# etrigger/Parsip

Measured on AMD Instinct MI355X. Metric: Mcells/sec polygonized, 256^3 grid 32-prim BlobTree, at 1/2/4/8 MI355X, higher is better.
Workload: dtype f32

## Files before the change

include/parsip_gpu.h:

```cpp
#ifndef PARSIP_GPU_H
#define PARSIP_GPU_H

#ifdef __HIPCC_RTC__
typedef __SIZE_TYPE__ size_t;
#ifndef offsetof
#define offsetof(t, m) __builtin_offsetof(t, m)
#endif
#else
#include <stddef.h>
#include <stdint.h>
#endif

#ifdef __cplusplus
extern "C" {
#endif

#define PSGPU_GRID_DIM              8
#define PSGPU_CELLS_PER_MPU         7
#define PSGPU_ISO_VALUE             0.5f
#define PSGPU_ISO_DIST              0.45420206f
#define PSGPU_NORMAL_DELTA          0.001f
#define PSGPU_MIN_CELL_SIZE         0.01f
#define PSGPU_MAX_TREE_NODES        128
#define PSGPU_PRIM_MATRIX_STRIDE    12
// ... 150 lines not shown
int  psgpu_weld_times(psgpu_ctx* ctx, float* ms, int maxPhases, const char** names);

int  psgpu_download_stats(psgpu_ctx* ctx, PsMpuStats* stats);
int  psgpu_export_polympus(psgpu_ctx* ctx, PsMPU* mpus, uint32_t capacity, uint32_t* outCtMPUs);
int  psgpu_polygonize_mpus(psgpu_ctx* ctx, float cellsize, const PsSoaBlobPrims* prims,
                           const PsSoaPrimMatrices* matrices, const PsSoaBlobOps* ops,
                           PsMPU* mpus, uint32_t capacity, uint32_t* outCtMPUs,
                           PsMpuStats* statsOrNull);
int  psgpu_polygonize_mpus_ex(psgpu_ctx* ctx, float cellsize, const PsSoaBlobPrims* prims,
                              const PsSoaPrimMatrices* matrices, const PsSoaBlobOps* ops,
                              PsMPU* mpus, uint32_t capacity, uint32_t* outCtMPUs,
                              PsMpuStats* statsOrNull, PsMpuProcessStats* processStatsOrNull);
int  psgpu_download_process_stats(psgpu_ctx* ctx, PsMpuProcessStats* out);
int  psgpu_download_stamps(psgpu_ctx* ctx, uint64_t* out, uint32_t* cap);
int  psgpu_vertex_queue(psgpu_ctx* ctx, uint32_t* counts, uint32_t* recs, uint32_t capacity);
int  psgpu_print_thread_results(int ctAttempts, uint32_t* lpThreadProcessed, uint32_t* lpThreadCrossed,
                                uint32_t capacity, int print);
int  psgpu_thread_result_count(void);
int  psgpu_last_kernel_times(psgpu_ctx* ctx, float* ms, int maxKernels, const char** names);
int  psgpu_field_values(psgpu_ctx* ctx, const float* xyz, uint32_t n, int mode, float* out, float* colOut);
int  psgpu_download_spans(psgpu_ctx* ctx, uint64_t* out, uint32_t* runs);

int  psgpu_set_option(psgpu_ctx* ctx, int option, int64_t value);
#define PSGPU_OPT_KERNEL_TIMING 1
#define PSGPU_OPT_CULLING       2
#define PSGPU_OPT_DEBUG         9
#define PSGPU_OPT_VERTEX_BLOCKS_PER_CU 4
#define PSGPU_OPT_FINISH_BLOCKS_PER_CU 5
#define PSGPU_OPT_GRAPH         7
#define PSGPU_OPT_CAPACITY      6
#define PSGPU_OPT_BOUND        10
#define PSGPU_OPT_JIT           3
#define PSGPU_OPT_TIER_RUNS    18
#define PSGPU_OPT_STAMPS       12
#define PSGPU_OPT_SPANS        13
#define PSGPU_OPT_FINISH_QUAD  14
#define PSGPU_OPT_VERTEX_WIDE  15
#define PSGPU_OPT_TREE_SPLIT   16
#define PSGPU_OPT_SPLIT_MAX_QUEUED 17
#define PSGPU_OPT_FUSED_SURFACE 21
// ... 101 lines not shown
```

parsip_amd/csrc/psgpu_device.h:

```cpp
#pragma once
#include "psgpu_model.h"

namespace psgpu {

typedef const __attribute__((address_space(4))) DevModel* ModelPtr;
typedef const __attribute__((address_space(4))) DevPrim CPrim;
typedef const __attribute__((address_space(4))) DevOp COp;
typedef const __attribute__((address_space(4))) CubeTablesDev* TablePtr;
__device__ __forceinline__ ModelPtr as_const(const DevModel* m) { return (ModelPtr)m; }
__device__ __forceinline__ TablePtr as_const(const CubeTablesDev* t) { return (TablePtr)t; }

__device__ __forceinline__ Instr load_instr(ModelPtr M, int pc) {
    typedef const __attribute__((address_space(4))) uint32_t* CU32;
    const CU32 w = (CU32)(&M->instr[pc]);
    const uint32_t words[3] = {w[0], w[1], w[2]};
    Instr I;
    __builtin_memcpy(&I, words, 12);
    return I;
}

__device__ __forceinline__ float max_ref(float a, float b) { return a > b ? a : b; }
__device__ __forceinline__ float min_ref(float a, float b) { return a < b ? a : b; }
__device__ __forceinline__ float m01(bool c) { return c ? 1.0f : 0.0f; }
__device__ __forceinline__ int lane_id() { return __lane_id(); }
// ... 260 lines not shown
    case PSGPU_T_UNION: case PSGPU_T_INTERSECT:
        *wl = m01((v - lf) == 0.0f);
        *wr = m01((v - rf) == 0.0f);
        return true;
    case PSGPU_T_DIF: case PSGPU_T_SMOOTHDIF:
        *wl = m01(lf == v);
        *wr = m01((1.0f - rf) == v);
        return true;
    default:
        return false;
    }
}

struct CullMask {
    uint64_t lo, hi;
};

struct CullLanes {
    CullSeg s[2];
    bool two;
};

__device__ __forceinline__ CullSeg load_cullseg(ModelPtr M, int i) {
    typedef const __attribute__((address_space(4))) float* CF;
    const CF f = (CF)(&M->cull[i]);
    CullSeg S;
    S.a[0] = f[0]; S.a[1] = f[1]; S.a[2] = f[2];
    S.u[0] = f[3]; S.u[1] = f[4]; S.u[2] = f[5];
    S.invUU = f[6]; S.radius = f[7];
    S.tmin = f[8]; S.tmax = f[9]; S.axisClear = f[10]; S.pad = f[11];
    return S;
// ... 485 lines not shown
    const bool vOf = __shfl(valid ? 1 : 0, lane * 8 & 63) != 0;
    const bool pass = lane < 8 && ((queue8 >> lane) & 1u);
    if (lane < 8 && vOf) {
        p.passed[mOf - p.mpuBegin] = (uint8_t)(((flags8 >> lane) & 1u) + ((queue8 >> lane) & 1u));
        if (!pass) p.counts[mOf - p.mpuBegin] = 0ull;
        if (p.mpuTicks) mpu_ticks_s1(p, mOf - p.mpuBegin, tick0);
    }
    if (flags8 == 0u) return;
    const uint32_t shard = W / (p.pShardCap / 8u);
    if (lane == 1 && proven8 != 0u) atomicAdd(&p.ctr->shard[shard].b, (uint32_t)__popc(proven8));
    if (queue8 == 0u) return;
    const uint32_t qsel = FRONT ? (blockIdx.x & 7u) : shard;
    const uint32_t qbase = FRONT ? qsel * p.fqCap : shard * p.pShardCap;
    uint32_t baseAtomic = 0;
    if (lane == 0) baseAtomic = atomicAdd(&p.ctr->shard[qsel].p, (uint32_t)__popc(queue8));
    uint64_t mLo = 0ull, mHi = 0ull;
    if (p.cull) {
        const float eg = 7.0f * p.cs + 0.001f;
        for (uint32_t qm = queue8; qm != 0u; qm &= qm - 1u) {
            const int q = __builtin_ctz(qm);
            const float ox = __int_as_float(__builtin_amdgcn_readlane(__float_as_int(o[0]), 8 * q));
            const float oy = __int_as_float(__builtin_amdgcn_readlane(__float_as_int(o[1]), 8 * q));
            const float oz = __int_as_float(__builtin_amdgcn_readlane(__float_as_int(o[2]), 8 * q));
            const CullMask g = cull_mask_from(cl, ox, oy, oz, ox + eg, oy + eg, oz + eg);
            const uint32_t wq = lane_value(mOf, q) - p.mpuBegin;
            if (lane == 0) {
                p.mpuMasks[2 * wq] = g.lo;
                p.mpuMasks[2 * wq + 1] = g.hi;
            }
            if (lane == q) {
                mLo = g.lo;
                mHi = g.hi;
            }
        }
    }
    asm volatile("" : "+v"(baseAtomic) : "v"(mLo));
    const uint32_t base = lane_value(baseAtomic, 0);
    if (pass) {
        const uint32_t slotq = qbase + base + (uint32_t)__popc(queue8 & ((1u << lane) - 1u));
        if (FRONT) {
            __hip_atomic_store(&p.pq[slotq], mOf, __ATOMIC_RELAXED, __HIP_MEMORY_SCOPE_AGENT);
            if (p.cull) {
                __hip_atomic_store(&p.pqMask[2 * slotq], mLo, __ATOMIC_RELAXED, __HIP_MEMORY_SCOPE_AGENT);
                __hip_atomic_store(&p.pqMask[2 * slotq + 1], mHi, __ATOMIC_RELAXED, __HIP_MEMORY_SCOPE_AGENT);
            }
        } else {
            p.pq[slotq] = mOf;
            if (p.cull) {
                p.pqMask[2 * slotq] = mLo;
                p.pqMask[2 * slotq + 1] = mHi;
            }
        }
    }
    phase_stamp(p, 3, 8192u);
    if constexpr (FRONT) {
        asm volatile("s_waitcnt vmcnt(0)" ::: "memory");
        if (pass) {
            const uint32_t slotq = qbase + base + (uint32_t)__popc(queue8 & ((1u << lane) - 1u));
            __hip_atomic_store(&p.fqReady[slotq], front_tag(p), __ATOMIC_RELAXED, __HIP_MEMORY_SCOPE_AGENT);
        }
    }
}

#ifndef PSGPU_S2_N
#define PSGPU_S2_N 8
// ... 95 lines not shown
        if (blk * (uint32_t)MPB >= pcount) return;
        live = d < pcount;
        if (live) {
            const uint32_t pshard = (uint32_t)__popcll(ballot(incl <= d));
            const uint32_t pidx = d - (pshard ? sIncl[pshard - 1] : 0u);
            slotq = uniform(pshard * p.pShardCap + pidx);
        }
    }
    uint32_t m = 0, w = 0;
    float o[3] = {0.0f, 0.0f, 0.0f};
    CullMask cm{0ull, 0ull};
    if (live) {
        if (FRONT) {
            m = uniform(__hip_atomic_load(&p.pq[slotq], __ATOMIC_RELAXED, __HIP_MEMORY_SCOPE_AGENT));
            if (p.cull) {
                cm.lo = uniform64(__hip_atomic_load(&p.pqMask[2 * slotq], __ATOMIC_RELAXED, __HIP_MEMORY_SCOPE_AGENT));
                cm.hi = uniform64(__hip_atomic_load(&p.pqMask[2 * slotq + 1], __ATOMIC_RELAXED, __HIP_MEMORY_SCOPE_AGENT));
            }
        } else {
            m = uniform(p.pq[slotq]);
            if (p.cull) {
                cm.lo = uniform64(p.pqMask[2 * slotq]);
                cm.hi = uniform64(p.pqMask[2 * slotq + 1]);
            }
        }
        *item = m;
        w = m - p.mpuBegin;
        mpu_origin(p, m, o);
    }
    phase_stamp(p, 1);
    unsigned char* base = smem + slot * kLdsMpu;
    uint16_t* edgeVid = reinterpret_cast<uint16_t*>(base + kLdsEdge);
    uint8_t* cellCfg = base + kLdsCfg;
    uint16_t* cellV = reinterpret_cast<uint16_t*>(base + kLdsVbase);
    uint16_t* cellT = reinterpret_cast<uint16_t*>(base + kLdsTbase);
    uint64_t* sIns = reinterpret_cast<uint64_t*>(base + kLdsIns);
    uint32_t* sQ = reinterpret_cast<uint32_t*>(base + kLdsQ);
    EV ev(M, reinterpret_cast<float*>(smem + kLdsWaveSlots + wave * p.slotsPerLane * 64 * 4) + lane);
// ... 361 lines not shown
#pragma unroll
        for (int i = 0; i < 8; ++i) {
            runV += (uint32_t)ch.c[i];
            runT += (uint32_t)(ch.c[i] >> 32);
            out[i] = (uint64_t)runV | ((uint64_t)runT << 32);
        }
#pragma unroll
        for (int i = 0; i < 8; ++i)
            if (e0 + i < hi) p.offs[e0 + i + 1] = out[i];
        carryV += totV;
        carryT += totT;
    }
}

__device__ __forceinline__ CullMask cull_mask_mpus(const Params& p, uint32_t w) {
    CullMask cm{~0ull, ~0ull};
    bool todo = true;
    for (;;) {
        const uint64_t b = ballot(todo);
        if (b == 0ull) break;
        const uint32_t w0 = lane_value(w, (int)__builtin_ctzll(b));
        cm.lo &= p.mpuMasks[2 * w0];
        cm.hi &= p.mpuMasks[2 * w0 + 1];
        if (w == w0) todo = false;
    }
    return cm;
}

struct EdgeSeg {
    float e[3], d[3];
};
__device__ __forceinline__ EdgeSeg edge_segment(const Params& p, uint32_t w, uint32_t key) {
    float o[3];
    mpu_origin(p, w + p.mpuBegin, o);
    const int sx = key & 7, sy = (key >> 3) & 7, sz = (key >> 6) & 7, ax = (key >> 9) & 3;
    const float cs = p.cs;
    EdgeSeg E;
    E.e[0] = o[0] + cs * (float)sx;
// ... 624 lines not shown
```

parsip_amd/csrc/psgpu_host.cpp:

```cpp
#include <hip/hip_runtime.h>

#include <atomic>
#include <algorithm>
#include <numeric>
#include <cmath>
#include <cstdio>
#include <cstdlib>
#include <cstring>
#include <ctime>
#include <functional>
#include <limits>
#include <memory>
#include <chrono>
#include <mutex>
#include <string>
#include <thread>
#include <vector>

#include "../../include/parsip_gpu.h"
#include "psgpu_internal.h"
#include "psgpu_launch.h"


using namespace psgpu;
// ... 368 lines not shown
    return (size_t)bd[0] * bd[1] * bd[2];
}

uint32_t front_sub_cap(uint32_t blocks, uint32_t mpb) { return 8u * mpb * ((blocks + 7u) / 8u); }
uint32_t front_cap(size_t bricks) {
    const uint32_t b = (uint32_t)bricks;
    return std::max(front_sub_cap((b + 1u) / 2u, 2u), front_sub_cap((b + 3u) / 4u, 4u));
}

int ensure_buffers(psgpu_ctx* c, uint32_t mpuCount) {
    const size_t n = std::max<uint32_t>(mpuCount, 1);
    c->pShardCap = 8u * (uint32_t)((brick_count(c) + kShards - 1) / kShards);
    const size_t fq = 8 * front_cap(brick_count(c));
    const size_t nq = std::max<size_t>((size_t)c->pShardCap * kShards, fq);
    PSGPU_CHECK(grow(c->pq, c->capList, nq));
    PSGPU_CHECK(grow(c->pqMask, c->capPqMask, nq * 2));
    if (fq > c->capFq) {
        PSGPU_CHECK(grow(c->fqReady, c->capFq, fq));
        PSGPU_CHECK(hipMemset(c->fqReady, 0, c->capFq * sizeof(uint32_t)));
    }
    PSGPU_CHECK(grow(c->counts, c->capCounts, n));
    PSGPU_CHECK(grow(c->passed, c->capPassed, n));
    PSGPU_CHECK(grow(c->mpuMasks, c->capMasks, 2 * n));
    PSGPU_CHECK(grow(c->offs, c->capOff, n + 1));
    PSGPU_CHECK(grow(c->vk, c->capVk, (size_t)c->vShardCap * kShards));
    PSGPU_CHECK(grow(c->vp, c->capVp, (size_t)c->vShardCap * kShards));
    PSGPU_CHECK(grow(c->tq, c->capTq, (size_t)c->tShardCap * kShards));
    size_t capV2 = c->capV, capV3 = c->capV;
    PSGPU_CHECK(grow(c->pos, c->capV, (size_t)c->vcap * 3));
    PSGPU_CHECK(grow(c->nrm, capV2, (size_t)c->vcap * 3));
    PSGPU_CHECK(grow(c->col, capV3, (size_t)c->vcap * 3));
    PSGPU_CHECK(grow(c->tris, c->capT, (size_t)c->tcap * 3));
    if (c->mpuTicksOpt) PSGPU_CHECK(grow(c->mpuTicks, c->capTicks, 4 * n));
    return PSGPU_RET_SUCCESS;
}

bool use_split(const psgpu_ctx* c) {
    if (!c->jit || !c->jit->precheckS || !c->splittable) return false;
// ... 42 lines not shown
    if (use_front(c)) {
        const uint32_t sub = !c->haveQueued ? p.fqCap
                             : (c->lastSubMax ? c->lastSubMax : (c->lastQueued + 7u) / 8u) + c->lastQueued / 32u + 32u;
        const uint32_t rows = (std::min(sub, p.fqCap) + mpb - 1u) / mpb;
        p.mpuBlocks = 8u * std::max(1u, rows);
    }
    if (c->debug & (1 << 20)) p.mpuBlocks = use_front(c) ? 8u : 1u;
    p.scanChunks = (c->mpuCount + kScanItems * kScanMaxBlocks - 1) / (kScanItems * kScanMaxBlocks);
    if (p.scanChunks == 0) p.scanChunks = 1;
    p.scanBlocks = (c->mpuCount + kScanItems * p.scanChunks - 1) / (kScanItems * p.scanChunks);
    p.scanStatus = c->scanStatus + (size_t)c->parity * kScanMaxBlocks;
    p.scanStatusNext = c->scanStatus + (size_t)(c->parity ^ 1u) * kScanMaxBlocks;
    p.counts = c->counts;
    p.passed = c->passed;
    p.bound = (c->bound && c->jit && c->model.boundable) ? 1u : 0u;
    p.mpuMasks = c->mpuMasks;
    p.offs = c->offs;
    p.vk = c->vk;
    p.vp = c->vp;
    p.vShardCap = c->vShardCap;
    p.tq = c->tq;
    p.tShardCap = c->tShardCap;
    p.pos = c->pos;
    p.nrm = c->nrm;
    p.col = c->col;
    p.tris = c->tris;
    p.vCap = c->vcap;
    p.tCap = c->tcap;
    p.ctr = c->ctr + c->parity;
    p.ctrNext = c->ctr + (c->parity ^ 1u);
// ... 472 lines not shown
            return PSGPU_RET_DEVICE_ERROR;
        }
    }
    {
        DevCounters init[2];
        memset(init, 0, sizeof(init));
        init[0].firstOverflow = init[1].firstOverflow = 0x7fffffff;
        if (hipMemcpy(c->ctr, init, sizeof(init), hipMemcpyHostToDevice) != hipSuccess) {
            psgpu_destroy(c);
            return PSGPU_RET_DEVICE_ERROR;
        }
    }
    for (int i = 0; i <= kNumKernels; ++i) (void)hipEventCreate(&c->ev[i]);
    const char* cullEnv = getenv("PSGPU_CULL");
    if (cullEnv) c->cull = atoi(cullEnv) != 0;
    const char* jitEnv = getenv("PSGPU_JIT");
    if (jitEnv) c->useJit = std::min(3, std::max(0, atoi(jitEnv)));
    const char* asyncEnv = getenv("PSGPU_JIT_ASYNC");
    if (asyncEnv) c->jitAsync = atoi(asyncEnv) != 0;
    if (const char* e = getenv("PSGPU_GRID_FIT")) c->gridFit = atoi(e) != 0;
    if (const char* e = getenv("PSGPU_FINISH_QUAD")) c->finishQuad = std::min(3, std::max(0, atoi(e)));
    if (const char* e = getenv("PSGPU_VERTEX_WIDE")) c->vertexWide = std::min(2, std::max(0, atoi(e)));
    if (const char* e = getenv("PSGPU_MPU_MARGIN")) c->mpuMarginDiv = std::max(1, atoi(e));
    if (const char* e = getenv("PSGPU_FUSED_SURFACE")) c->fusedSurface = std::min(3, std::max(0, atoi(e)));
    if (const char* e = getenv("PSGPU_FRONT")) c->front = std::min(2, std::max(0, atoi(e)));
    *out = c;
    return PSGPU_RET_SUCCESS;
}

void psgpu_destroy(psgpu_ctx* c) {
// ... 20 lines not shown
    if (c->hostStage) (void)hipHostFree(c->hostStage);
    for (int i = 0; i <= kNumKernels; ++i)
        if (c->ev[i]) (void)hipEventDestroy(c->ev[i]);
    for (hipEvent_t e : c->exportEv)
        if (e) (void)hipEventDestroy(e);
    if (c->stream) (void)hipStreamDestroy(c->stream);
    delete c;
}

int psgpu_set_option(psgpu_ctx* c, int option, int64_t value) {
    if (!c) return PSGPU_RET_PARAM_ERROR;
    const int drc = set_device(c);
    if (drc != PSGPU_RET_SUCCESS) return drc;
    if (option == PSGPU_OPT_KERNEL_TIMING) c->timing = value != 0;
    else if (option == PSGPU_OPT_CULLING) c->cull = value != 0;
    else if (option == PSGPU_OPT_DEBUG) c->debug = (int)value;
    else if (option == PSGPU_OPT_GRAPH) c->useGraph = value != 0;
    else if (option == PSGPU_OPT_BOUND) c->bound = value != 0;
    else if (option == PSGPU_OPT_CAPACITY && value >= 64 && value <= (1ll << 30)) {
        if (c->pending) (void)hipStreamSynchronize(c->runStream);
        set_pending(c, false);
        c->seenV = c->seenT = c->seenShardV = c->seenShardT = 0;
        void* bufs[] = {c->vk, c->vp, c->tq, c->pos, c->nrm, c->col, c->tris};
        for (void* b : bufs)
            if (b) (void)hipFree(b);
        c->vk = nullptr; c->vp = nullptr; c->tq = nullptr; c->pos = nullptr; c->nrm = nullptr; c->col = nullptr; c->tris = nullptr;
        c->capVk = c->capVp = c->capTq = c->capV = c->capT = 0;
        c->vcap = (uint32_t)value;
        c->tcap = (uint32_t)std::min<int64_t>(2 * value, 0xffffffffll);
        c->vShardCap = (uint32_t)std::max<int64_t>(16, value / kShards);
// ... 259 lines not shown
    if (rc != PSGPU_RET_SUCCESS) return rc;
    std::vector<VertexKey> shard;
    for (int k = 0; k < kShards; ++k) {
        if (counts[k] == 0) continue;
        shard.resize(counts[k]);
        PSGPU_CHECK(hipMemcpy(shard.data(), c->vk + (size_t)k * c->vShardCap, (size_t)counts[k] * sizeof(VertexKey),
                              hipMemcpyDeviceToHost));
        for (const VertexKey& K : shard) {
            *recs++ = K.w;
            *recs++ = K.vidKey & 0xffffu;
        }
    }
    return PSGPU_RET_SUCCESS;
}

int psgpu_download_spans(psgpu_ctx* c, uint64_t* out, uint32_t* runs) {
    if (!c || !runs) return PSGPU_RET_PARAM_ERROR;
    *runs = c->spans ? c->spanNext : 0u;
    if (!c->spans || !out || c->spanNext == 0) return PSGPU_RET_SUCCESS;
    int rc = set_device(c);
    if (rc != PSGPU_RET_SUCCESS) return rc;
    if (c->pending) PSGPU_CHECK(hipStreamSynchronize(c->runStream));
    const size_t per = (size_t)2 * kNumStampKernels * kSpanLanes;
    std::vector<uint64_t> raw((size_t)c->spanNext * per);
    PSGPU_CHECK(hipMemcpy(raw.data(), c->spans, raw.size() * 8, hipMemcpyDeviceToHost));
    for (uint32_t r = 0; r < c->spanNext; ++r)
        for (int k = 0; k < kNumStampKernels; ++k) {
            uint64_t lo = ~0ull, hi = 0ull;
            for (int l = 0; l < kSpanLanes; ++l) {
                const uint64_t* s = &raw[r * per + 2 * ((size_t)k * kSpanLanes + l)];
// ... 592 lines not shown
```

parsip_amd/csrc/psgpu_internal.h:

```cpp
#pragma once
#include <hip/hip_runtime.h>

#include <atomic>
#include <chrono>
#include <memory>
#include <string>
#include <vector>

#include "../../include/parsip_gpu.h"
#include "psgpu_jit.h"
#include "psgpu_model.h"
#include "psgpu_pool.h"

namespace psgpu {
constexpr int kNumKernels = 4;
}

namespace psgpu {
constexpr int kExportPieces = 16;
constexpr size_t kExportPieceBytes = 1u << 20;

constexpr int kWeldPhases = 6;
struct WeldState {
    unsigned char* table = nullptr;
// ... 85 lines not shown
    uint64_t* pqMask = nullptr;
    size_t capPqMask = 0;
    uint32_t pShardCap = 0;
    uint32_t lastQueued = 0;
    bool haveQueued = false;
    float lastCs = 0.0f;
    uint32_t runMpuBlocks = 0;
    uint64_t* scanStatus = nullptr;
    uint32_t parity = 0;
    uint64_t epochRuns = 0;
    uint64_t* counts = nullptr;
    uint8_t* passed = nullptr;
    size_t capPassed = 0;
    int bound = 1;
    uint64_t* mpuMasks = nullptr;
    size_t capMasks = 0;
    uint64_t* offs = nullptr;
    VertexKey* vk = nullptr;
    VertexPos* vp = nullptr;
    TriRec* tq = nullptr;
    float* pos = nullptr;
    float* nrm = nullptr;
    float* col = nullptr;
    uint32_t* tris = nullptr;
    DevCounters* ctr = nullptr;
    uint32_t* totals = nullptr;
    uint32_t* emptyTotals = nullptr;
    uint64_t* stamps = nullptr;
    uint32_t stampCap = 0;
    uint64_t* spans = nullptr;
// ... 83 lines not shown
```

parsip_amd/csrc/psgpu_jit.cpp:

```cpp
#include <hip/hip_runtime.h>
#include <hip/hiprtc.h>

#include <unistd.h>

#include <filesystem>
#include <future>

#include <cstdio>
#include <cstdlib>
#include <cstring>
#include <map>
#include <memory>
#include <mutex>
#include <sstream>
#include <string>
#include <vector>

#include "psgpu_jit.h"
#include "psgpu_model.h"

#include "_psgpu_embed.h"

namespace psgpu {
namespace {
// ... 180 lines not shown
        const Instr* I = op_instr(op);
        const int type = I->type, kind = I->childKind, L = I->L, R = I->R;
        const std::string v = "v" + std::to_string(op);
        o << "    float " << v << "[N], " << v << "c0[N], " << v << "c1[N], " << v << "c2[N];\n";
        o << FN("{ " + v + "c0[n] = 0.0f; " + v + "c1[n] = 0.0f; " + v + "c2[n] = 0.0f; }");
        if (zeroSkip) {
            emit_zero(op);
            o << "    if (!z" << op << ") {\n";
        }
        const bool groupRoot = emit_group(op, depth);
        std::string act = A;
        if (depth > 3) {
            const std::string b = "o" + std::to_string(op), a = "a" + std::to_string(op);
            o << "    {\n    " << (baked || opLoaded[op] ? "const BakedOp& " : "COp& ") << b << " = " << wop(op) << ";\n";
            const std::string in = "i" + std::to_string(op), lin = "l" + std::to_string(op);
            o << "    bool " << a << "[N], " << in << "[N];\n    bool any" << op << " = false, " << lin << " = false;\n";
            std::ostringstream s;
            o << FN(in + "[n] = ((px[n] >= " + b + ".lo[0]) & (" + b + ".hi[0] >= px[n])) | ((py[n] >= " + b +
                    ".lo[1]) & (" + b + ".hi[1] >= py[n])) | ((pz[n] >= " + b + ".lo[2]) & (" + b + ".hi[2] >= pz[n]));");
            o << "    if constexpr (GROUP == 0) {\n" << FN(lin + " |= (" + act_n(A) + ") && " + in + "[n];") << "    }\n";
            s << "{\n      const bool pr = (" << act_n(A) << ") && !(GROUP == 0 ? " << lin << " : group_any<GROUP>(("
              << act_n(A) << ") && " << in << "[n]));\n";
            if (trackLast) s << "      if (pr) last[n] = 0.0f;\n";
            s << "      " << a << "[n] = (" << act_n(A) << ") && !pr;\n";
            s << "      any" << op << " |= " << a << "[n];\n    }";
            o << FN(s.str());
            act = a;
            o << "    if (COLOR || ballot(any" << op << ") != 0ull) {\n";
        } else {
            o << "    {\n    {\n";
        }
        std::string rv, lv, rc[3], lc[3];
        if (kind & 1) {
            emit_op(R, depth + 1, act);
            rv = "v" + std::to_string(R) + "[n]";
            for (int k = 0; k < 3; ++k) rc[k] = "v" + std::to_string(R) + "c" + std::to_string(k) + "[n]";
        }
        if (kind & 2) {
            emit_op(L, depth + 1, act);
            lv = "v" + std::to_string(L) + "[n]";
            for (int k = 0; k < 3; ++k) lc[k] = "v" + std::to_string(L) + "c" + std::to_string(k) + "[n]";
// ... 257 lines not shown
                     "v0c2[n]; }\n    }");
    }
    o << "  }\n";
    o << "  template <int GROUP, bool COLOR>\n";
    o << "  __device__ __forceinline__ float eval(float px, float py, float pz, const CullMask& cm, float* colOut) "
         "const {\n    float r;\n    evaln<GROUP, COLOR, 1>(&px, &py, &pz, cm, &r, colOut);\n    return r;\n  }\n";
    g.emit_bound();
    g.emit_split();
    o << "};\n}  // namespace psgpu\n\n";
    const unsigned nopk = packed_fp32_policy(baked);
    static const char* kAttrs[8] = {"PSGPU_PRE_ATTR",  "PSGPU_MPU_ATTR",  "PSGPU_VTX_ATTR",  "PSGPU_FIN_ATTR",
                                    "PSGPU_PRES_ATTR", "PSGPU_MPUS_ATTR", "PSGPU_VTXQ_ATTR", "PSGPU_FINS_ATTR"};
    for (int k = 0; k < 8; ++k)
        o << "#ifndef " << kAttrs[k] << "\n#define " << kAttrs[k]
          << (((nopk >> k) & 1u) ? " __attribute__((target(\"no-packed-fp32-ops\")))" : "") << "\n#endif\n";
    o << "extern \"C\" __global__ void __launch_bounds__(256) PSGPU_PRE_ATTR jit_precheck(psgpu::Params p) {\n"
         "  extern __shared__ float lds[];\n"
         "  PSGPU_STAMPED(0, item_, psgpu::precheck_body<psgpu::TreeEval>(p, lds));\n}\n";
    o << "extern \"C\" __global__ void __launch_bounds__(256) PSGPU_MPU_ATTR jit_mpu(psgpu::Params p) {\n"
         "  extern __shared__ __attribute__((aligned(16))) unsigned char smem[];\n"
         "  PSGPU_STAMPED(1, item_, psgpu::mpu_body<psgpu::TreeEval>(p, smem, &item_));\n}\n";
    o << "extern \"C\" __global__ void __launch_bounds__(256) PSGPU_MPU_ATTR jit_front(psgpu::Params p) {\n"
         "  extern __shared__ __attribute__((aligned(16))) unsigned char smem[];\n"
         "  psgpu::front_body<psgpu::TreeEval, 1>(p, smem);\n}\n";
    if (split && g.splittable()) {
    o << "extern \"C\" __global__ void __launch_bounds__(256) PSGPU_PRES_ATTR jit_precheck_s(psgpu::Params p) {\n"
         "  extern __shared__ float lds[];\n"
         "  PSGPU_STAMPED(0, item_, (psgpu::precheck_body<psgpu::TreeEval, 2>(p, lds)));\n}\n";
    o << "extern \"C\" __global__ void __launch_bounds__(256) PSGPU_MPUS_ATTR jit_mpu_s(psgpu::Params p) {\n"
         "  extern __shared__ __attribute__((aligned(16))) unsigned char smem[];\n"
// ... 5 lines not shown
    if (split) {
    o << "extern \"C\" __global__ void __launch_bounds__(256) PSGPU_FIN_ATTR jit_surface_w(psgpu::Params p) {\n"
         "  extern __shared__ __attribute__((aligned(16))) float slds[];\n"
         "  PSGPU_STAMPED(3, item_, (psgpu::surface_body<psgpu::TreeEval, 64>(p, slds)));\n}\n";
    if (g.splittable())
    o << "extern \"C\" __global__ void __launch_bounds__(256) PSGPU_MPUS_ATTR jit_front_s(psgpu::Params p) {\n"
         "  extern __shared__ __attribute__((aligned(16))) unsigned char smem[];\n"
         "  psgpu::front_body<psgpu::TreeEval, 2>(p, smem);\n}\n";
    }
    o << "extern \"C\" __global__ void __launch_bounds__(256) PSGPU_VTXQ_ATTR jit_vertex(psgpu::Params p) {\n"
         "  extern __shared__ __attribute__((aligned(16))) float vlds[];\n"
         "  PSGPU_STAMPED(2, item_, (psgpu::vertex_body<psgpu::TreeEval, 16>(p, vlds)));\n}\n";
    o << "extern \"C\" __global__ void __launch_bounds__(256) PSGPU_VTX_ATTR jit_vertex_w(psgpu::Params p) {\n"
         "  extern __shared__ __attribute__((aligned(16))) float vlds[];\n"
         "  PSGPU_STAMPED(2, item_, (psgpu::vertex_body<psgpu::TreeEval, 64>(p, vlds)));\n}\n";
    o << "extern \"C\" __global__ void __launch_bounds__(256) PSGPU_FIN_ATTR jit_finish(psgpu::Params p) {\n"
         "  extern __shared__ __attribute__((aligned(16))) float flds[];\n"
         "  PSGPU_STAMPED(3, item_, (psgpu::finish_body<psgpu::TreeEval, 64>(p, flds)));\n}\n";
    o << "extern \"C\" __global__ void __launch_bounds__(256) PSGPU_FINS_ATTR jit_finish_q(psgpu::Params p) {\n"
         "  extern __shared__ __attribute__((aligned(16))) float flds[];\n"
         "  PSGPU_STAMPED(3, item_, (psgpu::finish_body<psgpu::TreeEval, 16>(p, flds)));\n}\n";
    o << "extern \"C\" __global__ void __launch_bounds__(256) PSGPU_FINS_ATTR jit_finish_p(psgpu::Params p) {\n"
         "  extern __shared__ __attribute__((aligned(16))) float flds[];\n"
         "  PSGPU_STAMPED(3, item_, (psgpu::finish_body<psgpu::TreeEval, 32>(p, flds)));\n}\n";
    o << "extern \"C\" __global__ void __launch_bounds__(256) jit_probe(psgpu::Params p, const float* xyz, float* "
         "out, float* colOut, uint32_t n, int mode) {\n"
         "  extern __shared__ __attribute__((aligned(16))) float plds[];\n"
         "  psgpu::probe_body<psgpu::TreeEval>(p, plds, xyz, out, colOut, n, mode);\n}\n";
    return o.str();
}

// ... 254 lines not shown
```

parsip_amd/csrc/psgpu_model.h:

```cpp
#pragma once
#ifdef __HIPCC_RTC__
typedef unsigned char uint8_t;
typedef signed char int8_t;
typedef unsigned short uint16_t;
typedef unsigned int uint32_t;
typedef int int32_t;
typedef unsigned long long uint64_t;
typedef long long int64_t;
#else
#include <stdint.h>
#include <hip/hip_runtime.h>
#endif

namespace psgpu {

#define PSGPU_T_CYLINDER 0
#define PSGPU_T_DISC 1
#define PSGPU_T_LINE 2
#define PSGPU_T_POINT 3
#define PSGPU_T_RING 4
#define PSGPU_T_CUBE 6
#define PSGPU_T_TRIANGLE 7
#define PSGPU_T_UNION 14
#define PSGPU_T_INTERSECT 15
#define PSGPU_T_DIF 16
#define PSGPU_T_SMOOTHDIF 17
#define PSGPU_T_BLEND 18
#define PSGPU_T_RICCI 19

// ... 126 lines not shown
    uint32_t mpuCount;
    uint32_t cull;
    uint32_t preBlocks;
    uint32_t brickI0;
    uint32_t brickDims[3];
    uint32_t brickStride;
    uint32_t* pq;
    uint64_t* pqMask;
    uint32_t pShardCap;
    uint32_t* fqReady;
    uint32_t fqCap;
    uint32_t mpuBlocks;
    uint64_t* counts;
    uint8_t* passed;
    uint32_t bound;
    uint64_t* mpuMasks;
    uint64_t* offs;
    uint64_t* scanStatus;
    uint64_t* scanStatusNext;
    uint32_t scanBlocks;
    uint32_t scanChunks;
    VertexKey* vk;
    VertexPos* vp;
    uint32_t vShardCap;
    TriRec* tq;
    uint32_t tShardCap;
    float* pos;
    float* nrm;
    float* col;
    uint32_t* tris;
// ... 15 lines not shown
```

parsip_amd/gpu.py:

```python
from __future__ import annotations

import atexit
import ctypes
import os
import threading
import weakref
from dataclasses import dataclass

import numpy as np

from . import soa

_LIB = None
_LIVE = weakref.WeakSet()
LIB_PATH = os.path.join(os.path.dirname(os.path.abspath(__file__)), "libparsip_gpu.so")
LIB_PATH = os.environ.get("PSGPU_AB_LIB") or LIB_PATH


class PsMeshInfo(ctypes.Structure):
    _fields_ = [("ctMPUs", ctypes.c_uint32), ("ctPassedPrecheck", ctypes.c_uint32),
                ("ctSurfaceMPUs", ctypes.c_uint32), ("ctVertices", ctypes.c_uint32),
                ("ctTriangles", ctypes.c_uint32), ("firstOverflowMPU", ctypes.c_int32),
                ("ctLaneEvals", ctypes.c_uint64), ("ctFieldMPUs", ctypes.c_uint32),
                ("launchFlags", ctypes.c_uint32)]
# ... 22 lines not shown
    "psgpu_count_mpus", "psgpu_mpu_dims", "psgpu_prepare_bboxes", "psgpu_translate_blobtree_type",
    "psgpu_tritable", "psgpu_version", "psgpu_create", "psgpu_destroy", "psgpu_device_count",
    "psgpu_set_model", "psgpu_polygonize", "psgpu_finish", "psgpu_mesh_device", "psgpu_download_mesh",
    "psgpu_download_stats", "psgpu_export_polympus", "psgpu_polygonize_mpus", "psgpu_last_kernel_times",
    "psgpu_field_values", "psgpu_set_option", "psgpu_jit_active", "psgpu_jit_source", "psgpu_jit_compile",
    "psgpu_jit_pending", "psgpu_jit_wait", "psgpu_jit_tier", "psgpu_mpu_costs", "psgpu_split_costs",
    "psgpu_group_create", "psgpu_group_destroy", "psgpu_group_size", "psgpu_group_context",
    "psgpu_group_set_option", "psgpu_group_set_model", "psgpu_group_jit_wait", "psgpu_group_set_split",
    "psgpu_group_get_split", "psgpu_group_polygonize", "psgpu_group_finish", "psgpu_group_download_mesh",
    "psgpu_group_gather", "psgpu_group_export_polympus", "psgpu_group_polygonize_mpus",
    "psgpu_comm_unique_id", "psgpu_comm_create", "psgpu_comm_destroy", "psgpu_comm_exchange",
    "psgpu_comm_result", "psgpu_download_stamps", "psgpu_comm_exchange_group", "psgpu_download_spans",
    "psgpu_comm_reexchanged", "psgpu_polygonize_mpus_ex", "psgpu_download_process_stats",
    "psgpu_print_thread_results", "psgpu_thread_result_count",
    "psgpu_weld", "psgpu_weld_device", "psgpu_download_weld", "psgpu_weld_times",
    "psgpu_vertex_queue",
]

OPT_KERNEL_TIMING = 1
OPT_CULLING = 2
OPT_JIT = 3
OPT_DEBUG = 9
OPT_VERTEX_BLOCKS_PER_CU = 4
OPT_FINISH_BLOCKS_PER_CU = 5
OPT_CAPACITY = 6
OPT_GRAPH = 7
OPT_BOUND = 10
OPT_JIT_ASYNC = 11
OPT_STAMPS = 12
OPT_SPANS = 13
OPT_FINISH_QUAD = 14
OPT_VERTEX_WIDE = 15
OPT_TREE_SPLIT = 16
OPT_SPLIT_MAX_QUEUED = 17
OPT_TIER_RUNS = 18
OPT_MPU_TICKS = 19
OPT_FUSED_SURFACE = 21
OPT_FRONT = 22
LAUNCH_TREE_SPLIT, LAUNCH_SURFACE, LAUNCH_FRONT, LAUNCH_RERUN = 1, 2, 4, 8
DEBUG_SURFACE_LATE_SCAN = 1 << 25
DEBUG_LOOKBACK_TIMEOUT = 1 << 26
DEBUG_FRONT_LATE_S1 = 1 << 27
DEBUG_EPOCH_NEAR_WRAP = 1 << 28
DEBUG_EXPORT_POISON = 1 << 23
DEBUG_EXPORT_STRAGGLER = 1 << 24
JIT_INTERP, JIT_STRUCTURE, JIT_BAKED, JIT_TIERED = 0, 1, 2, 3
STAMP_KERNELS = ("k_precheck", "k_mpu", "k_vertex", "k_finish")
GROUP_OPT_BALANCE = 100
GROUP_OPT_MIN_PART_MPUS = 101
BLOCKING_MIN_PART_MPUS = 16384
BALANCE_EVEN, BALANCE_PLAN, BALANCE_EVERY_RUN, BALANCE_FIXED = 0, 1, 2, 3
COMM_ID_BYTES = 128

# ... 57 lines not shown
        "psgpu_group_gather": ([vp, i32, ctypes.POINTER(PsMeshDevice)], i32),
        "psgpu_group_export_polympus": ([vp, vp, u32, ctypes.POINTER(u32)], i32),
        "psgpu_group_polygonize_mpus": ([vp, f32, vp, vp, vp, vp, u32, ctypes.POINTER(u32)], i32),
        "psgpu_comm_unique_id": ([vp], i32),
        "psgpu_comm_create": ([vp, vp, i32, i32, ctypes.POINTER(vp)], i32),
        "psgpu_comm_destroy": ([vp], None),
        "psgpu_comm_exchange": ([vp, vp], i32),
        "psgpu_comm_exchange_group": ([vp, vp], i32),
        "psgpu_comm_result": ([vp, ctypes.POINTER(PsMeshInfo), vp], i32),
        "psgpu_comm_reexchanged": ([vp], i32),
        "psgpu_weld": ([vp, ctypes.POINTER(PsWeldInfo)], i32),
        "psgpu_weld_device": ([vp, ctypes.POINTER(PsWeldDevice)], i32),
        "psgpu_download_weld": ([vp, vp, vp, vp, vp, vp], i32),
        "psgpu_weld_times": ([vp, vp, i32, vp], i32),
        "psgpu_vertex_queue": ([vp, vp, vp, u32], i32),
    }
    for name, (args, res) in sig.items():
        fn = getattr(L, name)
        fn.argtypes = args
        fn.restype = res
    _LIB = L
    return L


class PsgpuError(RuntimeError):
    def __init__(self, code: int, what: str):
        super().__init__(f"{what} failed with code {code}")
        self.code = code


# ... 171 lines not shown

    def stats(self) -> np.ndarray:
        info = self.finish()
        st = np.zeros(info.ctMPUs, soa.MPU_STATS_DTYPE)
        _check(self._L.psgpu_download_stats(self._ctx, st.ctypes.data), "psgpu_download_stats")
        return st

    def vertex_queue(self) -> tuple[np.ndarray, list[np.ndarray]]:
        info = self.finish()
        counts = np.zeros(64, np.uint32)
        recs = np.zeros((max(info.ctVertices, 1), 2), np.uint32)
        _check(self._L.psgpu_vertex_queue(self._ctx, counts.ctypes.data, recs.ctypes.data, len(recs)),
               "psgpu_vertex_queue")
        ends = np.cumsum(counts.astype(np.int64))
        return counts, [recs[e - n:e] for e, n in zip(ends, counts.astype(np.int64))]

    def export_polympus(self, capacity: int | None = None) -> np.ndarray:
        info = self.finish()
        cap = info.ctMPUs if capacity is None else capacity
        out = np.zeros(max(cap, 1), soa.MPU_DTYPE)
        ct = ctypes.c_uint32()
        _check(self._L.psgpu_export_polympus(self._ctx, out.ctypes.data, cap, ctypes.byref(ct)),
               "psgpu_export_polympus")
        return out[:ct.value]

    def polygonize_mpus(self, cellsize: float, model: soa.Model, poly_mpus: np.ndarray | None = None,
                        stats: np.ndarray | None = None, process_stats: np.ndarray | None = None):
        if poly_mpus is None:
            poly_mpus = np.zeros(soa.MAX_MPU_COUNT, soa.MPU_DTYPE)
        ct = ctypes.c_uint32()
# ... 320 lines not shown
```

Before: 334,700.

## Precompute per-MPU op-box containment masks to skip per-point range tests

During precheck, each queued MPU now gets a per-operator 'fully inside the op's bounding slab' bitmask, built with a wave ballot. The mask is stored next to the existing cull masks, which doubles the mask buffers to four words per entry. The JIT-generated evaluator checks this bit and skips the per-point lo/hi range tests and proof logic for operators whose range trivially covers the MPU. It also caps SGPRs on the non-baked finish kernel. The cost is extra mask memory traffic and ballot work in precheck, plus a risk of register pressure from the SGPR cap.

```diff
diff --git a/include/parsip_gpu.h b/include/parsip_gpu.h
--- a/include/parsip_gpu.h
+++ b/include/parsip_gpu.h
@@ -188,6 +188,7 @@
 int  psgpu_download_process_stats(psgpu_ctx* ctx, PsMpuProcessStats* out);
 int  psgpu_download_stamps(psgpu_ctx* ctx, uint64_t* out, uint32_t* cap);
 int  psgpu_vertex_queue(psgpu_ctx* ctx, uint32_t* counts, uint32_t* recs, uint32_t capacity);
+int  psgpu_mpu_masks(psgpu_ctx* ctx, uint8_t* queued, uint64_t* masks, uint32_t capacity);
 int  psgpu_print_thread_results(int ctAttempts, uint32_t* lpThreadProcessed, uint32_t* lpThreadCrossed,
                                 uint32_t capacity, int print);
 int  psgpu_thread_result_count(void);
@@ -198,6 +199,7 @@
 int  psgpu_set_option(psgpu_ctx* ctx, int option, int64_t value);
 #define PSGPU_OPT_KERNEL_TIMING 1
 #define PSGPU_OPT_CULLING       2
+#define PSGPU_OPT_OP_INSIDE    23
 #define PSGPU_OPT_DEBUG         9
 #define PSGPU_OPT_VERTEX_BLOCKS_PER_CU 4
 #define PSGPU_OPT_FINISH_BLOCKS_PER_CU 5
diff --git a/parsip_amd/csrc/psgpu_device.h b/parsip_amd/csrc/psgpu_device.h
--- a/parsip_amd/csrc/psgpu_device.h
+++ b/parsip_amd/csrc/psgpu_device.h
@@ -298,7 +298,11 @@
 
 struct CullMask {
     uint64_t lo, hi;
+    uint64_t inLo, inHi;
 };
+__device__ __forceinline__ bool op_inside(const CullMask& cm, uint32_t k) {
+    return k < 64 ? ((cm.inLo >> k) & 1ull) : ((cm.inHi >> (k - 64)) & 1ull);
+}
 
 struct CullLanes {
     CullSeg s[2];
@@ -814,23 +818,42 @@
     const uint32_t qbase = FRONT ? qsel * p.fqCap : shard * p.pShardCap;
     uint32_t baseAtomic = 0;
     if (lane == 0) baseAtomic = atomicAdd(&p.ctr->shard[qsel].p, (uint32_t)__popc(queue8));
-    uint64_t mLo = 0ull, mHi = 0ull;
+    uint64_t mLo = 0ull, mHi = 0ull, iLo = 0ull, iHi = 0ull;
     if (p.cull) {
         const float eg = 7.0f * p.cs + 0.001f;
+        ModelPtr Mo = as_const(p.model);
+        const uint32_t nOps = p.opInside ? Mo->ctOps : 0u;
+        float bl[2][3], bh[2][3];
+#pragma unroll
+        for (int h = 0; h < 2; ++h) {
+            const uint32_t k = 64u * h + (uint32_t)lane;
+#pragma unroll
+            for (int a = 0; a < 3; ++a) {
+                bl[h][a] = k < nOps ? p.model->ops[k].lo[a] : 1.0f;
+                bh[h][a] = k < nOps ? p.model->ops[k].hi[a] : -1.0f;
+            }
+        }
         for (uint32_t qm = queue8; qm != 0u; qm &= qm - 1u) {
             const int q = __builtin_ctz(qm);
             const float ox = __int_as_float(__builtin_amdgcn_readlane(__float_as_int(o[0]), 8 * q));
             const float oy = __int_as_float(__builtin_amdgcn_readlane(__float_as_int(o[1]), 8 * q));
             const float oz = __int_as_float(__builtin_amdgcn_readlane(__float_as_int(o[2]), 8 * q));
-            const CullMask g = cull_mask_from(cl, ox, oy, oz, ox + eg, oy + eg, oz + eg);
+            CullMask g = cull_mask_from(cl, ox, oy, oz, ox + eg, oy + eg, oz + eg);
+            if (nOps != 0u) g.inLo = ballot((uint32_t)lane < nOps && op_inside_box(bl[0], bh[0], ox, oy, oz, p.cs));
+            if (nOps > 64u)
+                g.inHi = ballot(64u + (uint32_t)lane < nOps && op_inside_box(bl[1], bh[1], ox, oy, oz, p.cs));
             const uint32_t wq = lane_value(mOf, q) - p.mpuBegin;
             if (lane == 0) {
-                p.mpuMasks[2 * wq] = g.lo;
-                p.mpuMasks[2 * wq + 1] = g.hi;
+                p.mpuMasks[4 * wq] = g.lo;
+                p.mpuMasks[4 * wq + 1] = g.hi;
+                p.mpuMasks[4 * wq + 2] = g.inLo;
+                p.mpuMasks[4 * wq + 3] = g.inHi;
             }
             if (lane == q) {
                 mLo = g.lo;
                 mHi = g.hi;
+                iLo = g.inLo;
+                iHi = g.inHi;
             }
         }
     }
@@ -841,14 +864,18 @@
         if (FRONT) {
             __hip_atomic_store(&p.pq[slotq], mOf, __ATOMIC_RELAXED, __HIP_MEMORY_SCOPE_AGENT);
             if (p.cull) {
-                __hip_atomic_store(&p.pqMask[2 * slotq], mLo, __ATOMIC_RELAXED, __HIP_MEMORY_SCOPE_AGENT);
-                __hip_atomic_store(&p.pqMask[2 * slotq + 1], mHi, __ATOMIC_RELAXED, __HIP_MEMORY_SCOPE_AGENT);
+                __hip_atomic_store(&p.pqMask[4 * slotq], mLo, __ATOMIC_RELAXED, __HIP_MEMORY_SCOPE_AGENT);
+                __hip_atomic_store(&p.pqMask[4 * slotq + 1], mHi, __ATOMIC_RELAXED, __HIP_MEMORY_SCOPE_AGENT);
+                __hip_atomic_store(&p.pqMask[4 * slotq + 2], iLo, __ATOMIC_RELAXED, __HIP_MEMORY_SCOPE_AGENT);
+                __hip_atomic_store(&p.pqMask[4 * slotq + 3], iHi, __ATOMIC_RELAXED, __HIP_MEMORY_SCOPE_AGENT);
             }
         } else {
             p.pq[slotq] = mOf;
             if (p.cull) {
-                p.pqMask[2 * slotq] = mLo;
-                p.pqMask[2 * slotq + 1] = mHi;
+                p.pqMask[4 * slotq] = mLo;
+                p.pqMask[4 * slotq + 1] = mHi;
+                p.pqMask[4 * slotq + 2] = iLo;
+                p.pqMask[4 * slotq + 3] = iHi;
             }
         }
     }
@@ -974,14 +1001,19 @@
         if (FRONT) {
             m = uniform(__hip_atomic_load(&p.pq[slotq], __ATOMIC_RELAXED, __HIP_MEMORY_SCOPE_AGENT));
             if (p.cull) {
-                cm.lo = uniform64(__hip_atomic_load(&p.pqMask[2 * slotq], __ATOMIC_RELAXED, __HIP_MEMORY_SCOPE_AGENT));
-                cm.hi = uniform64(__hip_atomic_load(&p.pqMask[2 * slotq + 1], __ATOMIC_RELAXED, __HIP_MEMORY_SCOPE_AGENT));
+                cm.lo = uniform64(__hip_atomic_load(&p.pqMask[4 * slotq], __ATOMIC_RELAXED, __HIP_MEMORY_SCOPE_AGENT));
+                cm.hi = uniform64(__hip_atomic_load(&p.pqMask[4 * slotq + 1], __ATOMIC_RELAXED, __HIP_MEMORY_SCOPE_AGENT));
+                cm.inLo = uniform64(__hip_atomic_load(&p.pqMask[4 * slotq + 2], __ATOMIC_RELAXED, __HIP_MEMORY_SCOPE_AGENT));
+                if (M->ctOps > 64u)
+                    cm.inHi = uniform64(__hip_atomic_load(&p.pqMask[4 * slotq + 3], __ATOMIC_RELAXED, __HIP_MEMORY_SCOPE_AGENT));
             }
         } else {
             m = uniform(p.pq[slotq]);
             if (p.cull) {
-                cm.lo = uniform64(p.pqMask[2 * slotq]);
-                cm.hi = uniform64(p.pqMask[2 * slotq + 1]);
+                cm.lo = uniform64(p.pqMask[4 * slotq]);
+                cm.hi = uniform64(p.pqMask[4 * slotq + 1]);
+                cm.inLo = uniform64(p.pqMask[4 * slotq + 2]);
+                cm.inHi = uniform64(p.pqMask[4 * slotq + 3]);
             }
         }
         *item = m;
@@ -1373,14 +1405,16 @@
 }
 
 __device__ __forceinline__ CullMask cull_mask_mpus(const Params& p, uint32_t w) {
-    CullMask cm{~0ull, ~0ull};
+    CullMask cm{~0ull, ~0ull, ~0ull, ~0ull};
     bool todo = true;
     for (;;) {
         const uint64_t b = ballot(todo);
         if (b == 0ull) break;
         const uint32_t w0 = lane_value(w, (int)__builtin_ctzll(b));
-        cm.lo &= p.mpuMasks[2 * w0];
-        cm.hi &= p.mpuMasks[2 * w0 + 1];
+        cm.lo &= p.mpuMasks[4 * w0];
+        cm.hi &= p.mpuMasks[4 * w0 + 1];
+        cm.inLo &= p.mpuMasks[4 * w0 + 2];
+        cm.inHi &= p.mpuMasks[4 * w0 + 3];
         if (w == w0) todo = false;
     }
     return cm;
diff --git a/parsip_amd/csrc/psgpu_host.cpp b/parsip_amd/csrc/psgpu_host.cpp
--- a/parsip_amd/csrc/psgpu_host.cpp
+++ b/parsip_amd/csrc/psgpu_host.cpp
@@ -406,14 +406,14 @@
     const size_t fq = 8 * front_cap(brick_count(c));
     const size_t nq = std::max<size_t>((size_t)c->pShardCap * kShards, fq);
     PSGPU_CHECK(grow(c->pq, c->capList, nq));
-    PSGPU_CHECK(grow(c->pqMask, c->capPqMask, nq * 2));
+    PSGPU_CHECK(grow(c->pqMask, c->capPqMask, nq * 4));
     if (fq > c->capFq) {
         PSGPU_CHECK(grow(c->fqReady, c->capFq, fq));
         PSGPU_CHECK(hipMemset(c->fqReady, 0, c->capFq * sizeof(uint32_t)));
     }
     PSGPU_CHECK(grow(c->counts, c->capCounts, n));
     PSGPU_CHECK(grow(c->passed, c->capPassed, n));
-    PSGPU_CHECK(grow(c->mpuMasks, c->capMasks, 2 * n));
+    PSGPU_CHECK(grow(c->mpuMasks, c->capMasks, 4 * n));
     PSGPU_CHECK(grow(c->offs, c->capOff, n + 1));
     PSGPU_CHECK(grow(c->vk, c->capVk, (size_t)c->vShardCap * kShards));
     PSGPU_CHECK(grow(c->vp, c->capVp, (size_t)c->vShardCap * kShards));
@@ -486,6 +486,7 @@
     p.counts = c->counts;
     p.passed = c->passed;
     p.bound = (c->bound && c->jit && c->model.boundable) ? 1u : 0u;
+    p.opInside = c->opInside ? 1u : 0u;
     p.mpuMasks = c->mpuMasks;
     p.offs = c->offs;
     p.vk = c->vk;
@@ -988,6 +989,7 @@
     for (int i = 0; i <= kNumKernels; ++i) (void)hipEventCreate(&c->ev[i]);
     const char* cullEnv = getenv("PSGPU_CULL");
     if (cullEnv) c->cull = atoi(cullEnv) != 0;
+    if (const char* e = getenv("PSGPU_OP_INSIDE")) c->opInside = atoi(e) != 0;
     const char* jitEnv = getenv("PSGPU_JIT");
     if (jitEnv) c->useJit = std::min(3, std::max(0, atoi(jitEnv)));
     const char* asyncEnv = getenv("PSGPU_JIT_ASYNC");
@@ -1038,6 +1040,7 @@
     if (drc != PSGPU_RET_SUCCESS) return drc;
     if (option == PSGPU_OPT_KERNEL_TIMING) c->timing = value != 0;
     else if (option == PSGPU_OPT_CULLING) c->cull = value != 0;
+    else if (option == PSGPU_OPT_OP_INSIDE) c->opInside = value != 0;
     else if (option == PSGPU_OPT_DEBUG) c->debug = (int)value;
     else if (option == PSGPU_OPT_GRAPH) c->useGraph = value != 0;
     else if (option == PSGPU_OPT_BOUND) c->bound = value != 0;
@@ -1327,6 +1330,25 @@
     return PSGPU_RET_SUCCESS;
 }
 
+int psgpu_mpu_masks(psgpu_ctx* c, uint8_t* queued, uint64_t* masks, uint32_t capacity) {
+    if (!c || !queued || !masks) return PSGPU_RET_PARAM_ERROR;
+    int rc = psgpu_finish(c, nullptr);
+    if (rc != PSGPU_RET_SUCCESS) return rc;
+    if (c->mpuCount > capacity) return PSGPU_RET_PARAM_ERROR;
+    if (c->mpuCount == 0) return PSGPU_RET_SUCCESS;
+    rc = set_device(c);
+    if (rc != PSGPU_RET_SUCCESS) return rc;
+    const size_t n = c->mpuCount;
+    PSGPU_CHECK(hipMemcpy(queued, c->passed, n, hipMemcpyDeviceToHost));
+    PSGPU_CHECK(hipMemcpy(masks, c->mpuMasks, 4 * n * sizeof(uint64_t), hipMemcpyDeviceToHost));
+    for (size_t w = 0; w < n; ++w) {
+        queued[w] = queued[w] == 2 ? 1 : 0;
+        if (!queued[w] || !c->cull)
+            for (int k = 0; k < 4; ++k) masks[4 * w + k] = 0ull;
+    }
+    return PSGPU_RET_SUCCESS;
+}
+
 int psgpu_download_spans(psgpu_ctx* c, uint64_t* out, uint32_t* runs) {
     if (!c || !runs) return PSGPU_RET_PARAM_ERROR;
     *runs = c->spans ? c->spanNext : 0u;
diff --git a/parsip_amd/csrc/psgpu_internal.h b/parsip_amd/csrc/psgpu_internal.h
--- a/parsip_amd/csrc/psgpu_internal.h
+++ b/parsip_amd/csrc/psgpu_internal.h
@@ -123,6 +123,7 @@
     size_t capPassed = 0;
     int bound = 1;
     uint64_t* mpuMasks = nullptr;
+    bool opInside = true;
     size_t capMasks = 0;
     uint64_t* offs = nullptr;
     VertexKey* vk = nullptr;
diff --git a/parsip_amd/csrc/psgpu_jit.cpp b/parsip_amd/csrc/psgpu_jit.cpp
--- a/parsip_amd/csrc/psgpu_jit.cpp
+++ b/parsip_amd/csrc/psgpu_jit.cpp
@@ -218,7 +218,11 @@
             const std::string b = "o" + std::to_string(op), a = "a" + std::to_string(op);
             o << "    {\n    " << (baked || opLoaded[op] ? "const BakedOp& " : "COp& ") << b << " = " << wop(op) << ";\n";
             const std::string in = "i" + std::to_string(op), lin = "l" + std::to_string(op);
-            o << "    bool " << a << "[N], " << in << "[N];\n    bool any" << op << " = false, " << lin << " = false;\n";
+            o << "    bool " << a << "[N];\n    bool any" << op << " = false;\n";
+            o << "    if (op_inside(cm, " << op << "u)) {\n"
+              << FN("{ " + a + "[n] = (" + act_n(A) + "); any" + std::to_string(op) + " |= " + a + "[n]; }")
+              << "    } else {\n";
+            o << "    bool " << in << "[N];\n    bool " << lin << " = false;\n";
             std::ostringstream s;
             o << FN(in + "[n] = ((px[n] >= " + b + ".lo[0]) & (" + b + ".hi[0] >= px[n])) | ((py[n] >= " + b +
                     ".lo[1]) & (" + b + ".hi[1] >= py[n])) | ((pz[n] >= " + b + ".lo[2]) & (" + b + ".hi[2] >= pz[n]));");
@@ -229,6 +233,7 @@
             s << "      " << a << "[n] = (" << act_n(A) << ") && !pr;\n";
             s << "      any" << op << " |= " << a << "[n];\n    }";
             o << FN(s.str());
+            o << "    }\n";
             act = a;
             o << "    if (COLOR || ballot(any" << op << ") != 0ull) {\n";
         } else {
@@ -516,6 +521,8 @@
     for (int k = 0; k < 8; ++k)
         o << "#ifndef " << kAttrs[k] << "\n#define " << kAttrs[k]
           << (((nopk >> k) & 1u) ? " __attribute__((target(\"no-packed-fp32-ops\")))" : "") << "\n#endif\n";
+    o << "#ifndef PSGPU_FIN_SGPR\n#define PSGPU_FIN_SGPR" << (baked ? "" : " __attribute__((amdgpu_num_sgpr(96)))")
+      << "\n#endif\n";
     o << "extern \"C\" __global__ void __launch_bounds__(256) PSGPU_PRE_ATTR jit_precheck(psgpu::Params p) {\n"
          "  extern __shared__ float lds[];\n"
          "  PSGPU_STAMPED(0, item_, psgpu::precheck_body<psgpu::TreeEval>(p, lds));\n}\n";
@@ -551,7 +558,7 @@
     o << "extern \"C\" __global__ void __launch_bounds__(256) PSGPU_VTX_ATTR jit_vertex_w(psgpu::Params p) {\n"
          "  extern __shared__ __attribute__((aligned(16))) float vlds[];\n"
          "  PSGPU_STAMPED(2, item_, (psgpu::vertex_body<psgpu::TreeEval, 64>(p, vlds)));\n}\n";
-    o << "extern \"C\" __global__ void __launch_bounds__(256) PSGPU_FIN_ATTR jit_finish(psgpu::Params p) {\n"
+    o << "extern \"C\" __global__ void __launch_bounds__(256) PSGPU_FIN_ATTR PSGPU_FIN_SGPR jit_finish(psgpu::Params p) {\n"
          "  extern __shared__ __attribute__((aligned(16))) float flds[];\n"
          "  PSGPU_STAMPED(3, item_, (psgpu::finish_body<psgpu::TreeEval, 64>(p, flds)));\n}\n";
     o << "extern \"C\" __global__ void __launch_bounds__(256) PSGPU_FINS_ATTR jit_finish_q(psgpu::Params p) {\n"
diff --git a/parsip_amd/csrc/psgpu_model.h b/parsip_amd/csrc/psgpu_model.h
--- a/parsip_amd/csrc/psgpu_model.h
+++ b/parsip_amd/csrc/psgpu_model.h
@@ -7,12 +7,31 @@
 typedef int int32_t;
 typedef unsigned long long uint64_t;
 typedef long long int64_t;
+#elif defined(PSGPU_MODEL_NO_HIP)
+#include <stdint.h>
 #else
 #include <stdint.h>
 #include <hip/hip_runtime.h>
 #endif
+#if defined(__HIPCC__) || defined(__HIPCC_RTC__)
+#define PSGPU_HD __host__ __device__
+#else
+#define PSGPU_HD
+#endif
 
 namespace psgpu {
+
+PSGPU_HD inline bool op_inside_axis(float opLo, float opHi, float o, float cs) {
+    const float hi = o + 7.0f * cs;
+    const float mag = __builtin_fmaxf(__builtin_fabsf(o), __builtin_fabsf(hi));
+    if (!(mag < 1e30f)) return false;
+    const float m = 0.002f + 1e-5f * mag;
+    return opLo <= o - m && hi + m <= opHi;
+}
+PSGPU_HD inline bool op_inside_box(const float opLo[3], const float opHi[3], float ox, float oy, float oz, float cs) {
+    return op_inside_axis(opLo[0], opHi[0], ox, cs) || op_inside_axis(opLo[1], opHi[1], oy, cs) ||
+           op_inside_axis(opLo[2], opHi[2], oz, cs);
+}
 
 #define PSGPU_T_CYLINDER 0
 #define PSGPU_T_DISC 1
@@ -169,6 +188,7 @@
     uint64_t* counts;
     uint8_t* passed;
     uint32_t bound;
+    uint32_t opInside;
     uint64_t* mpuMasks;
     uint64_t* offs;
     uint64_t* scanStatus;
diff --git a/parsip_amd/gpu.py b/parsip_amd/gpu.py
--- a/parsip_amd/gpu.py
+++ b/parsip_amd/gpu.py
@@ -60,7 +60,7 @@
     "psgpu_comm_reexchanged", "psgpu_polygonize_mpus_ex", "psgpu_download_process_stats",
     "psgpu_print_thread_results", "psgpu_thread_result_count",
     "psgpu_weld", "psgpu_weld_device", "psgpu_download_weld", "psgpu_weld_times",
-    "psgpu_vertex_queue",
+    "psgpu_vertex_queue", "psgpu_mpu_masks",
 ]
 
 OPT_KERNEL_TIMING = 1
@@ -83,6 +83,7 @@
 OPT_MPU_TICKS = 19
 OPT_FUSED_SURFACE = 21
 OPT_FRONT = 22
+OPT_OP_INSIDE = 23
 LAUNCH_TREE_SPLIT, LAUNCH_SURFACE, LAUNCH_FRONT, LAUNCH_RERUN = 1, 2, 4, 8
 DEBUG_SURFACE_LATE_SCAN = 1 << 25
 DEBUG_LOOKBACK_TIMEOUT = 1 << 26
@@ -170,6 +171,7 @@
         "psgpu_download_weld": ([vp, vp, vp, vp, vp, vp], i32),
         "psgpu_weld_times": ([vp, vp, i32, vp], i32),
         "psgpu_vertex_queue": ([vp, vp, vp, u32], i32),
+        "psgpu_mpu_masks": ([vp, vp, vp, u32], i32),
     }
     for name, (args, res) in sig.items():
         fn = getattr(L, name)
@@ -371,6 +373,14 @@
                "psgpu_vertex_queue")
         ends = np.cumsum(counts.astype(np.int64))
         return counts, [recs[e - n:e] for e, n in zip(ends, counts.astype(np.int64))]
+
+    def mpu_masks(self) -> tuple[np.ndarray, np.ndarray]:
+        info = self.finish()
+        queued = np.zeros(max(info.ctMPUs, 1), np.uint8)
+        masks = np.zeros((max(info.ctMPUs, 1), 4), np.uint64)
+        _check(self._L.psgpu_mpu_masks(self._ctx, queued.ctypes.data, masks.ctypes.data, len(queued)),
+               "psgpu_mpu_masks")
+        return queued[:info.ctMPUs].astype(bool), masks[:info.ctMPUs]
 
     def export_polympus(self, capacity: int | None = None) -> np.ndarray:
         info = self.finish()
```

New measurement: 349,800 (median of 6 runs). 4.5% higher.
